# anxingle/AlphaPig

Hardware: AMD Instinct MI355X
Metric: self-play games/sec (15x15, n_playout=400) (higher is better)
Workload: dtype f32 (split operands on the bf16/fp16 matrix pipe, fp32 accumulate; <=1e-4 vs float64 oracle)

## Files before the change

alphapig_amd/csrc/apz_engine.hip:

```cpp
#include <hip/hip_runtime.h>

#include <algorithm>
#include <cmath>
#include <cstdio>
#include <cstdlib>
#include <cstring>
#include <map>
#include <mutex>
#include <string>
#include <vector>

#include "alphapig_hip.h"
#include "conv3x3_mfma.h"
#include "heads.h"
#include "trunk15_ring.h"
#include "trunk15_wino3.h"
#include "trunk15_wino3s.h"
#include "trunk15_wino3b.h"
#include "trunk15_wino3h.h"
#include "trunk15_wino3h16.h"
#include "conv8_split.h"
#include "conv8_small.h"
#include "wgrad_wino3.h"
#include "sampler.h"
// ... 35 lines not shown
    bool residual;
    float* wpk = nullptr;
    float* wpk12 = nullptr;
    float* upk2 = nullptr;
    float* upk3s = nullptr;
    void* upk3b = nullptr;
    void* upk3h = nullptr;
    float* bias3h = nullptr;
    void* wpk8h = nullptr;
    float* bias8h = nullptr;
    float* bias = nullptr;
};

struct Pending {
    int cls;
    hipEvent_t a, b;
    int launches;
};

}

struct apz_engine {
    apz_config cfg;
    int hw = 0, code_stride = 0, num_cu = 256, cmax = 0, clast = 0;
    hipStream_t stream = nullptr;
    std::vector<Param> params;
    std::vector<ConvLayer> convs;
    bool loaded = false;
    float *w6 = nullptr, *b6 = nullptr, *wfc_pk = nullptr, *bfc = nullptr, *wv = nullptr, *bv = nullptr;
    float* act[3] = {nullptr, nullptr, nullptr};
    float *planes = nullptr, *featp = nullptr, *featv = nullptr, *probs = nullptr, *values = nullptr, *fc_logits = nullptr;
    unsigned char* codes = nullptr;
    int *perm_s = nullptr, *perm_p = nullptr;
    float *h_planes = nullptr, *h_probs = nullptr, *h_values = nullptr;
    unsigned char* h_codes = nullptr;
    int last_n = 0;
    struct Slot {
        unsigned char* h_codes = nullptr;
        float *h_probs = nullptr, *h_values = nullptr;
        float *d_probs = nullptr, *d_values = nullptr;
        unsigned char* d_codes = nullptr;
        hipEvent_t done = nullptr;
        int n = 0;
        bool busy = false;
    } slots[APZ_MAX_SLOTS];
    std::map<long, hipGraphExec_t> fwd_graphs;
    std::map<long, int> fwd_seen;
    bool use_graphs = false;
    std::recursive_mutex submit_lock;
    bool ring = false;
    bool small8 = false;
    float* wfc_raw = nullptr;
    int act_ps = 0, act_rs = 0;
    bool lds_attr_set[44] = {false};
    int conv_lds_set[16] = {0};
    int32_t* smp_vis = nullptr;
    float* smp_pi = nullptr;
    int32_t* smp_mv = nullptr;
    uint64_t* smp_keys = nullptr;
    size_t smp_cap = 0;
    float* zeros256 = nullptr;
    double* bn_part = nullptr;
    float* wgw_scratch = nullptr;
    double* fold_ws = nullptr;
    float* head_scratch = nullptr;
    size_t head_scratch_floats = 0;
    size_t wgw_floats = 0;
    void* adam_tab = nullptr;
    size_t adam_cap = 0;
    float* wino_scratch[2] = {nullptr, nullptr};
    size_t wino_scratch_boards = 0;
    bool wgrad_attr_set[2] = {false, false};
    hipStream_t scratch_stream = nullptr;
    bool scratch_stream_valid = false;
    float* w3s_slabs = nullptr;
    unsigned* w3s_tickets = nullptr;
    unsigned w3s_epoch = 0;
    bool no_small_trunk = false;
    bool no_quarter_trunk = false;
    int trunk_arith = APZ_ARITH_F32;
    unsigned* ovf_host = nullptr;
    unsigned* ovf_dev = nullptr;
    unsigned* ovf_cur = nullptr;
    bool force_f32 = false;
    bool f16x2_k8 = false;
    long ovf_repeats = 0;
    int trunk_kernel = APZ_TRUNK_WINOGRAD;
    bool profiling = false;
    int prof_stride = 1, prof_phase = 0;
    bool prof_now = false;
    std::vector<Pending> pending;
    std::vector<hipEvent_t> free_events;
    double k_ms[APZ_K_COUNT] = {0};
    long k_cnt[APZ_K_COUNT] = {0};
};

namespace {

void add_param(apz_engine* e, const std::string& n, int64_t sz) { e->params.push_back({n, sz}); }

void build_tables(apz_engine* e) {
    const apz_config& c = e->cfg;
    const int hw = e->hw;
    auto conv_act = [&](const std::string& name, int cin, int cout, int k) {
        add_param(e, name + "_weight", (int64_t)cout * cin * k * k);
        add_param(e, name + "_bias", cout);
        add_param(e, name + "_gamma", cout);
        add_param(e, name + "_beta", cout);
        add_param(e, name + "_mean", cout);
        add_param(e, name + "_var", cout);
    };
    int last = 0;
    if (c.net_kind == APZ_NET_RESNET) {
        const int F = c.n_filter;
        conv_act("res_conv1", c.c_in, F, 3);
        e->convs.push_back({"res_conv1", "res_conv1", "_mean", "_var", true, c.c_in, (c.c_in + 3) / 4 * 4, F, false});
        for (int i = 1; i <= c.n_blocks; i++) {
            for (const char* ab : {"A", "B"}) {
                const std::string cn = std::string("conv") + ab + std::to_string(i);
                const std::string bn = std::string("bn") + ab + std::to_string(i);
                add_param(e, cn + "_weight", (int64_t)F * F * 9);
                add_param(e, cn + "_bias", F);
                add_param(e, bn + "_gamma", F);
                add_param(e, bn + "_beta", F);
                add_param(e, bn + "_moving_mean", F);
                add_param(e, bn + "_moving_var", F);
                e->convs.push_back({cn, bn, "_moving_mean", "_moving_var", false, F, F, F, ab[0] == 'B'});
            }
        }
        last = F;
    } else {
        static const char* names[6] = {"conv1", "conv2", "conv3", "conv4", "conv5", "conv_final"};
        static const int widths[6] = {64, 64, 128, 128, 256, 256};
        int prev = c.c_in;
        for (int i = 0; i < 6; i++) {
            conv_act(names[i], prev, widths[i], 3);
            e->convs.push_back({names[i], names[i], "_mean", "_var", true, prev, (prev + 3) / 4 * 4, widths[i], false});
            prev = widths[i];
// ... 168 lines not shown
        configured = true;
    }
    if (upk_small && n <= apz::Wino3S::MAX_BOARDS && !e->no_small_trunk) {
        if (!e->w3s_slabs) {
            HIP_TRY(hipMalloc((void**)&e->w3s_slabs, apz::Wino3S::slab_floats() * sizeof(float)));
            HIP_TRY(hipMalloc((void**)&e->w3s_tickets, apz::Wino3S::counters() * sizeof(unsigned)));
            e->w3s_epoch = 0;
        }
        if (++e->w3s_epoch == 0 || e->w3s_epoch == 1) {
            e->w3s_epoch = 1;
            HIP_TRY(hipMemsetAsync(e->w3s_tickets, 0, apz::Wino3S::counters() * sizeof(unsigned), e->stream));
        }
        hipLaunchKernelGGL((apz::trunk15_wino3s_kernel<RESID, RELU>), dim3(n * 16), dim3(256), apz::Wino3S::LDS_BYTES, e->stream, in,
                           upk_small, bias, RESID ? resid : nullptr, out, n, e->w3s_slabs, e->w3s_tickets, e->w3s_epoch);
        HIP_TRY(hipGetLastError());
        return APZ_OK;
    }
    for (int b0 = 0; b0 < n; b0 += WINO3_MAX_BOARDS) {
        const int nb = std::min(n - b0, WINO3_MAX_BOARDS);
        const size_t off = (size_t)b0 * T::C * T::GPLANE;
        bool quarter = false;
        const int grid = apz::wino3_grid(nb, e->num_cu, e->no_quarter_trunk ? nullptr : &quarter);
        if (quarter)
            hipLaunchKernelGGL((apz::trunk15_wino3_kernel<RESID, RELU, true>), dim3(grid), dim3(512), T::LDS_BYTES, e->stream,
                               in + off, upk, bias, RESID ? resid + off : nullptr, out + off, nb);
        else
            hipLaunchKernelGGL((apz::trunk15_wino3_kernel<RESID, RELU>), dim3(grid), dim3(512), T::LDS_BYTES, e->stream, in + off,
                               upk, bias, RESID ? resid + off : nullptr, out + off, nb);
    }
    HIP_TRY(hipGetLastError());
    return APZ_OK;
}

template <bool RESID>
int launch_wino3b_t(apz_engine* e, int attr_slot, const ConvLayer& L, const float* in, const float* resid, float* out, int n) {
    using T = apz::Wino3B;
    bool& configured = e->lds_attr_set[attr_slot];
    if (!configured) {
        HIP_TRY(hipFuncSetAttribute((const void*)apz::trunk15_wino3b_kernel<RESID, true>, hipFuncAttributeMaxDynamicSharedMemorySize,
                                    T::LDS_BYTES));
        configured = true;
    }
    for (int b0 = 0; b0 < n; b0 += WINO3_MAX_BOARDS) {
        const int nb = std::min(n - b0, WINO3_MAX_BOARDS);
        const size_t off = (size_t)b0 * T::C * T::GPLANE;
        const int grid = apz::wino3_grid(nb, e->num_cu);
        hipLaunchKernelGGL((apz::trunk15_wino3b_kernel<RESID, true>), dim3(grid), dim3(512), T::LDS_BYTES, e->stream, in + off,
                           (const void*)L.upk3b, L.bias, RESID ? resid + off : nullptr, out + off, nb);
    }
    HIP_TRY(hipGetLastError());
    return APZ_OK;
}

template <bool RESID, bool K16>
int launch_wino3h_t(apz_engine* e, int attr_slot, const ConvLayer& L, const float* in, const float* resid, float* out, int n) {
    using T = typename std::conditional<K16, apz::Wino3H16, apz::Wino3H>::type;
    const void* kern = K16 ? (const void*)apz::trunk15_wino3h16_kernel<RESID, true> : (const void*)apz::trunk15_wino3h_kernel<RESID, true>;
    bool& configured = e->lds_attr_set[attr_slot];
    if (!configured) {
        HIP_TRY(hipFuncSetAttribute(kern, hipFuncAttributeMaxDynamicSharedMemorySize, T::LDS_BYTES));
        configured = true;
    }
    for (int b0 = 0; b0 < n; b0 += WINO3_MAX_BOARDS) {
        const int nb = std::min(n - b0, WINO3_MAX_BOARDS);
        const size_t off = (size_t)b0 * T::C * T::GPLANE;
        const int grid = apz::wino3_grid(nb, e->num_cu);
        if constexpr (K16)
            hipLaunchKernelGGL((apz::trunk15_wino3h16_kernel<RESID, true>), dim3(grid), dim3(512), T::LDS_BYTES, e->stream, in + off,
                               (const void*)L.upk3h, L.bias3h, RESID ? resid + off : nullptr, out + off, nb, e->ovf_cur, nullptr, 0);
        else
            hipLaunchKernelGGL((apz::trunk15_wino3h_kernel<RESID, true>), dim3(grid), dim3(512), T::LDS_BYTES, e->stream, in + off,
                               (const void*)L.upk3h, L.bias3h, RESID ? resid + off : nullptr, out + off, nb, e->ovf_cur);
    }
    HIP_TRY(hipGetLastError());
    return APZ_OK;
}

int launch_trunk_wino3(apz_engine* e, const ConvLayer& L, const float* in, const float* resid, float* out, int n) {
    if (e->trunk_arith == APZ_ARITH_F16X2 && !e->force_f32 && L.upk3h && e->ovf_cur &&
        (n > apz::Wino3S::MAX_BOARDS || e->no_small_trunk)) {
        if (e->f16x2_k8) {
            if (resid) return launch_wino3h_t<true, false>(e, 32, L, in, resid, out, n);
            return launch_wino3h_t<false, false>(e, 33, L, in, resid, out, n);
        }
        if (resid) return launch_wino3h_t<true, true>(e, 36, L, in, resid, out, n);
        return launch_wino3h_t<false, true>(e, 37, L, in, resid, out, n);
    }
    if (e->trunk_arith == APZ_ARITH_BF16X3 && L.upk3b && (n > apz::Wino3S::MAX_BOARDS || e->no_small_trunk)) {
        if (resid) return launch_wino3b_t<true>(e, 26, L, in, resid, out, n);
        return launch_wino3b_t<false>(e, 27, L, in, resid, out, n);
    }
    if (resid) return launch_wino3_t<true, true>(e, 6, in, L.upk2, L.bias, resid, out, n, L.upk3s);
    return launch_wino3_t<false, true>(e, 7, in, L.upk2, L.bias, nullptr, out, n, L.upk3s);
}

int launch_trunk_ring(apz_engine* e, const ConvLayer& L, const float* in, const float* resid, float* out, int n) {
    if (e->trunk_kernel == APZ_TRUNK_WINOGRAD && L.upk2) return launch_trunk_wino3(e, L, in, resid, out, n);
    return launch_trunk_ring_t<4>(e, L, in, resid, out, n);
}

template <int C4, int CIN, bool CODES>
int launch_stem15_t(apz_engine* e, const ConvLayer& L, const float* in, float* out, int n) {
    constexpr int lds = apz::stem15_lds_bytes<C4>();
    bool& configured = e->lds_attr_set[(C4 == 1 ? 2 : 3) + (CODES ? 22 : 0)];
    if (!configured) {
        HIP_TRY(hipFuncSetAttribute((const void*)apz::stem15_kernel<C4, CIN, CODES>, hipFuncAttributeMaxDynamicSharedMemorySize,
                                    lds));
        configured = true;
    }
    const int grid = std::min(n, e->num_cu * (C4 == 1 ? 4 : 2));
    hipLaunchKernelGGL((apz::stem15_kernel<C4, CIN, CODES>), dim3(grid), dim3(256), lds, e->stream, in, L.wpk, L.bias, out, n,
                       L.cin, (int)e->code_stride);
    HIP_TRY(hipGetLastError());
    return APZ_OK;
}

int launch_stem15(apz_engine* e, const ConvLayer& L, const float* in, float* out, int n, const unsigned char* codes = nullptr) {
    if (codes) {
        if (L.cin == 4) return launch_stem15_t<1, 4, true>(e, L, (const float*)codes, out, n);
        if (L.cin == 9) return launch_stem15_t<3, 9, true>(e, L, (const float*)codes, out, n);
    } else {
        if (L.cin == 4) return launch_stem15_t<1, 4, false>(e, L, in, out, n);
        if (L.cin == 9) return launch_stem15_t<3, 9, false>(e, L, in, out, n);
    }
    return fail(APZ_E_UNSUPPORTED, "stem15: C_in must be 4 or 9");
}

template <bool RESID, bool CODES>
int launch_conv8_t(apz_engine* e, const ConvLayer& L, const float* in, const float* resid, float* out, int n) {
    using T = apz::Conv8;
    bool& configured = e->lds_attr_set[28 + (RESID ? 1 : 0) + (CODES ? 2 : 0)];
    if (!configured) {
        HIP_TRY(hipFuncSetAttribute((const void*)apz::conv8_kernel<RESID, CODES>, hipFuncAttributeMaxDynamicSharedMemorySize,
                                    T::LDS_BYTES));
        configured = true;
    }
    const long items = (long)n * (L.cout / 16);
    const int grid = (int)std::min<long>(items, 2L * e->num_cu);
// ... 254 lines not shown
    }
    void* host[] = {e->h_planes, e->h_probs, e->h_values, e->h_codes};
    for (void* p : host)
        if (p) hipHostFree(p);
    if (e->stream) hipStreamDestroy(e->stream);
    delete e;
}

apz_engine* apz_create(const apz_config* cfg) {
    if (!cfg || cfg->height < 1 || cfg->width < 1 || cfg->max_batch < 1 || (cfg->c_in != 9 && cfg->c_in != 4)) {
        fail(APZ_E_ARG, "bad config (c_in must be 9 or 4)");
        return nullptr;
    }
    if (!((cfg->height == 15 && cfg->width == 15) || (cfg->height == 8 && cfg->width == 8))) {
        fail(APZ_E_UNSUPPORTED, "HIP kernels are instantiated for 15x15 and 8x8 boards");
        return nullptr;
    }
    if (cfg->net_kind == APZ_NET_RESNET &&
        ((cfg->n_filter != 64 && cfg->n_filter != 128 && cfg->n_filter != 256) || cfg->n_blocks < 0)) {
        fail(APZ_E_UNSUPPORTED, "n_filter must be 64, 128 or 256");
        return nullptr;
    }
    if (cfg->net_kind != APZ_NET_RESNET && cfg->net_kind != APZ_NET_SIMPLE) {
        fail(APZ_E_ARG, "unknown net_kind");
        return nullptr;
    }
    int ndev = 0;
    if (hipGetDeviceCount(&ndev) != hipSuccess || ndev < 1) {
        fail(APZ_E_HIP, "no HIP device: libalphapig_hip needs an AMD GPU (there is no CPU fallback)");
        return nullptr;
    }
    if (cfg->device < 0 || cfg->device >= ndev) {
        fail(APZ_E_ARG, "device ordinal out of range");
        return nullptr;
    }
    apz_engine* e = new apz_engine();
    e->cfg = *cfg;
    e->hw = cfg->height * cfg->width;
    e->code_stride = (e->hw + 1 + 15) / 16 * 16;
    build_tables(e);
    auto bail = [&](const char* what, hipError_t err) -> apz_engine* {
        fail(APZ_E_HIP, std::string(what) + ": " + hipGetErrorString(err));
        apz_destroy(e);
        return nullptr;
    };
    hipError_t err;
    if ((err = hipSetDevice(cfg->device)) != hipSuccess) return bail("hipSetDevice", err);
    hipDeviceProp_t prop;
    if ((err = hipGetDeviceProperties(&prop, cfg->device)) != hipSuccess) return bail("hipGetDeviceProperties", err);
    e->num_cu = prop.multiProcessorCount > 0 ? prop.multiProcessorCount : 256;
    {
        const char* k8 = getenv("APZ_F16X2_K8");
        e->f16x2_k8 = k8 && atoi(k8) != 0;
    }
    if ((err = hipStreamCreateWithFlags(&e->stream, hipStreamNonBlocking)) != hipSuccess)
        return bail("hipStreamCreate", err);
    e->ring = cfg->net_kind == APZ_NET_RESNET && cfg->height == 15 && cfg->width == 15 && cfg->n_filter == 128;
    e->small8 = cfg->height == 8 && cfg->width == 8;
    e->act_ps = e->ring ? apz::Trunk15::GPLANE : e->hw;
    e->act_rs = e->ring ? apz::Trunk15::GROW : cfg->width;
    const size_t B = cfg->max_batch, hw = e->hw;
    const size_t act_bytes = B * e->cmax * (size_t)e->act_ps * sizeof(float);
    for (int i = 0; i < 3; i++)
    {
        if ((err = hipMalloc((void**)&e->act[i], act_bytes)) != hipSuccess) return bail("hipMalloc(act)", err);
        if ((err = hipMemset(e->act[i], 0, act_bytes)) != hipSuccess) return bail("hipMemset(act)", err);
    }
    if ((err = hipMalloc((void**)&e->planes, B * 9 * hw * sizeof(float))) != hipSuccess) return bail("hipMalloc", err);
    if ((err = hipMalloc((void**)&e->featp, B * 4 * hw * sizeof(float))) != hipSuccess) return bail("hipMalloc", err);
    if ((err = hipMalloc((void**)&e->featv, B * 2 * hw * sizeof(float))) != hipSuccess) return bail("hipMalloc", err);
    if ((err = hipMalloc((void**)&e->probs, B * hw * sizeof(float))) != hipSuccess) return bail("hipMalloc", err);
    if ((err = hipMalloc((void**)&e->fc_logits, B * ((hw + 15) / 16 * 16) * sizeof(float))) != hipSuccess) return bail("hipMalloc", err);
    if ((err = hipMalloc((void**)&e->values, B * sizeof(float))) != hipSuccess) return bail("hipMalloc", err);
    if ((err = hipMalloc((void**)&e->codes, B * e->code_stride)) != hipSuccess) return bail("hipMalloc", err);
    if ((err = hipMemset(e->codes, 0, B * e->code_stride)) != hipSuccess) return bail("hipMemset(codes)", err);
    if ((err = hipHostMalloc((void**)&e->h_planes, B * 9 * hw * sizeof(float))) != hipSuccess) return bail("hipHostMalloc", err);
    if ((err = hipHostMalloc((void**)&e->h_probs, B * hw * sizeof(float))) != hipSuccess) return bail("hipHostMalloc", err);
    if ((err = hipHostMalloc((void**)&e->h_values, B * sizeof(float))) != hipSuccess) return bail("hipHostMalloc", err);
    if ((err = hipHostMalloc((void**)&e->h_codes, B * e->code_stride)) != hipSuccess) return bail("hipHostMalloc", err);
    if (cfg->height == cfg->width) {
        std::vector<int> ps, pp;
        build_perms(cfg->height, ps, pp);
        if (upload(&e->perm_s, ps) || upload(&e->perm_p, pp)) {
            apz_destroy(e);
            return nullptr;
        }
    }
    return e;
}

int apz_param_count(apz_engine* e) { return e ? (int)e->params.size() : fail(APZ_E_ARG, "null engine"); }

const char* apz_param_name(apz_engine* e, int i) {
    if (!e || i < 0 || i >= (int)e->params.size()) return nullptr;
    return e->params[i].name.c_str();
}

int64_t apz_param_size(apz_engine* e, int i) {
    if (!e || i < 0 || i >= (int)e->params.size()) return -1;
    return e->params[i].size;
}

int apz_load_weights(apz_engine* e, const char* const* names, const float* const* ptrs, const int64_t* sizes, int n) {
    if (!e || !names || !ptrs || !sizes) return fail(APZ_E_ARG, "null argument");
    EngineLock guard(e->submit_lock);
    HIP_TRY(hipSetDevice(e->cfg.device));
// ... 667 lines not shown
    if (!e || !x_dev || !upk_dev || !y_dev || !stats_dev || n < 1) return fail(APZ_E_ARG, "bad argument");
    if (e->cfg.height != 15 || e->cfg.width != 15) return fail(APZ_E_UNSUPPORTED, "wino_conv: 15x15 boards only");
    if (n > WINO3_MAX_BOARDS) return fail(APZ_E_UNSUPPORTED, "wino_conv_stats: one launch (<= 16384 boards)");
    using T = apz::Wino3;
    EngineLock guard(e->submit_lock);
    HIP_TRY(hipSetDevice(e->cfg.device));
    if (!e->zeros256) {
        HIP_TRY(hipMalloc((void**)&e->zeros256, 256 * sizeof(float)));
        HIP_TRY(hipMemset(e->zeros256, 0, 256 * sizeof(float)));
    }
    StreamScope sc(e, stream);
    bool& configured = e->lds_attr_set[11];
    if (!configured) {
        HIP_TRY(hipFuncSetAttribute((const void*)apz::trunk15_wino3_kernel<false, false, false, true>,
                                    hipFuncAttributeMaxDynamicSharedMemorySize, T::LDS_BYTES));
        HIP_TRY(hipFuncSetAttribute((const void*)apz::trunk15_wino3_kernel<false, false, true, true>,
                                    hipFuncAttributeMaxDynamicSharedMemorySize, T::LDS_BYTES));
        configured = true;
    }
    const float* b = bias_dev ? (const float*)bias_dev : e->zeros256;
    bool quarter = false;
    const int grid = apz::wino3_grid(n, e->num_cu, e->no_quarter_trunk ? nullptr : &quarter);
    if (quarter)
        hipLaunchKernelGGL((apz::trunk15_wino3_kernel<false, false, true, true>), dim3(grid), dim3(512), T::LDS_BYTES, e->stream,
                           (const float*)x_dev, (const float*)upk_dev, b, (const float*)stats_dev, (float*)y_dev, n);
    else
        hipLaunchKernelGGL((apz::trunk15_wino3_kernel<false, false, false, true>), dim3(grid), dim3(512), T::LDS_BYTES, e->stream,
                           (const float*)x_dev, (const float*)upk_dev, b, (const float*)stats_dev, (float*)y_dev, n);
    HIP_TRY(hipGetLastError());
    return APZ_OK;
}

int apz_wino_conv(apz_engine* e, const void* x_dev, const void* upk_dev, const void* bias_dev, void* y_dev, int n, int relu,
                  int layout, void* stream) {
    return apz_wino_conv_add(e, x_dev, upk_dev, bias_dev, nullptr, y_dev, n, relu, layout, stream);
}

int64_t apz_wino3h_packed_size(void) { return (int64_t)(apz::Wino3H16::UPK_BYTES / 4); }

int apz_wino3h_pack_many(apz_engine* e, const void* w_dev, const void* b_dev, int count, void* upk_dev, void* bias_dev,
                         void* flag_dev, void* stream) {
    if (!e || !w_dev || !upk_dev || !bias_dev || count < 1 || count > 16384) return fail(APZ_E_ARG, "bad argument");
    EngineLock guard(e->submit_lock);
    HIP_TRY(hipSetDevice(e->cfg.device));
    StreamScope sc(e, stream);
    hipLaunchKernelGGL(apz::pack_wino3h16_many_kernel, dim3(128, 2 * count), dim3(128), 0, e->stream, (const float*)w_dev,
                       (const float*)b_dev, (unsigned short*)upk_dev, (float*)bias_dev, (unsigned*)flag_dev);
    HIP_TRY(hipGetLastError());
    return APZ_OK;
}

extern "C++" {
namespace {
template <int FORM, bool RESID>
int launch_wino3h16_train(apz_engine* e, int attr_slot, const void* x_dev, const void* upk_dev, const void* bias_dev,
                          const void* resid_dev, void* y_dev, int n, void* flag_dev, void* aux, int aux_n, void* stream) {
    if (!e || !x_dev || !upk_dev || !bias_dev || !y_dev || !aux || n < 1) return fail(APZ_E_ARG, "bad argument");
    if (e->cfg.height != 15 || e->cfg.width != 15) return fail(APZ_E_UNSUPPORTED, "wino3h: 15x15 boards only");
    if (n > WINO3_MAX_BOARDS) return fail(APZ_E_UNSUPPORTED, "wino3h: one launch (<= 16384 boards)");
    using T = apz::Wino3H16;
    const auto kern = apz::trunk15_wino3h16_kernel<RESID, false, FORM>;
    EngineLock guard(e->submit_lock);
    HIP_TRY(hipSetDevice(e->cfg.device));
    StreamScope sc(e, stream);
    bool& configured = e->lds_attr_set[attr_slot];
    if (!configured) {
        HIP_TRY(hipFuncSetAttribute((const void*)kern, hipFuncAttributeMaxDynamicSharedMemorySize, T::LDS_BYTES));
        configured = true;
    }
    hipLaunchKernelGGL(kern, dim3(apz::wino3_grid(n, e->num_cu)), dim3(512), T::LDS_BYTES, e->stream, (const float*)x_dev, upk_dev,
                       (const float*)bias_dev, (const float*)resid_dev, (float*)y_dev, n, (unsigned*)flag_dev, aux, aux_n);
    HIP_TRY(hipGetLastError());
    return APZ_OK;
}
}
}

int apz_wino3h_conv_stats(apz_engine* e, const void* x_dev, const void* upk_dev, const void* bias_dev, void* y_dev,
                          void* stats_dev, int n, void* flag_dev, void* stream) {
    return launch_wino3h16_train<apz::WINO3H16_STATS, false>(e, 40, x_dev, upk_dev, bias_dev, nullptr, y_dev, n, flag_dev,
                                                             stats_dev, 0, stream);
}

int apz_wino3h_conv_dgrad(apz_engine* e, const void* dy_dev, const void* upk_dev, const void* bias_dev, const void* add_dev,
                          void* dx_dev, int n, const void* dymax_dev, int dymax_count, void* flag_dev, void* stream) {
    if (dymax_count < 1) return fail(APZ_E_ARG, "bad argument");
    void* dm = const_cast<void*>(dymax_dev);
    if (add_dev)
        return launch_wino3h16_train<apz::WINO3H16_DGRAD, true>(e, 41, dy_dev, upk_dev, bias_dev, add_dev, dx_dev, n, flag_dev, dm,
                                                                dymax_count, stream);
    return launch_wino3h16_train<apz::WINO3H16_DGRAD, false>(e, 42, dy_dev, upk_dev, bias_dev, nullptr, dx_dev, n, flag_dev, dm,
                                                             dymax_count, stream);
}

namespace {
int wgrad_scratch(apz_engine* e, size_t floats) {
    if (floats > e->wgw_floats) {
        HIP_TRY(hipDeviceSynchronize());
        if (e->wgw_scratch) HIP_TRY(hipFree(e->wgw_scratch));
        e->wgw_scratch = nullptr;
        e->wgw_floats = 0;
        HIP_TRY(hipMalloc((void**)&e->wgw_scratch, floats * sizeof(float)));
        e->wgw_floats = floats;
    }
    return APZ_OK;
}
}

int apz_conv3x3_wgrad(apz_engine* e, const void* x_dev, const void* dy_dev, void* dw_dev, int n, int cin, int cout,
                      int layout, void* stream) {
    if (!e || !x_dev || !dy_dev || !dw_dev || n < 1 || cin < 1 || cout < 32 || cout % 32 || layout < 0 || layout > 1)
        return fail(APZ_E_ARG, "bad argument (C_out must be a multiple of 32)");
    if (layout == APZ_LAYOUT_ROWS16 && (e->cfg.height != 15 || e->cfg.width != 15))
        return fail(APZ_E_UNSUPPORTED, "padded-row layout: 15x15 boards only");
    EngineLock guard(e->submit_lock);
    HIP_TRY(hipSetDevice(e->cfg.device));
    StreamScope sc(e, stream);
    const int H = e->cfg.height, W = e->cfg.width;
    const int gx = cout / 32, gy = (cin + 63) / 64;
    int slices = std::max(1, std::min(n, (e->num_cu * 2) / std::max(1, gx * gy)));
    if (H == 15 && W == 15) {
        using G = apz::WgradGeo<15, 15>;
        if (!e->wgrad_attr_set[0]) {
            HIP_TRY(hipFuncSetAttribute((const void*)apz::conv3x3_wgrad_kernel<15, 15>,
                                        hipFuncAttributeMaxDynamicSharedMemorySize, G::LDS_BYTES));
            e->wgrad_attr_set[0] = true;
// ... 611 lines not shown
```

alphapig_amd/csrc/trunk15_wino3h16.h:

```cpp
#pragma once
#include <hip/hip_runtime.h>

#include <cmath>
#include <cstdint>
#include <type_traits>

#include "trunk15_wino3h.h"

namespace apz {

struct Wino3H16 {
    static constexpr int C = 128, CK = 16, NCHUNK = C / CK;
    static constexpr int GPLANE = 240;
    static constexpr int VTERM = 32 * 32, VPOS = 2 * VTERM, V_BYTES = 36 * VPOS;
    static constexpr int UNIT = 2 * 32 * 16;
    static constexpr size_t UPK_BYTES = (size_t)4 * 4 * NCHUNK * 9 * 2 * UNIT;
    static constexpr int BIAS_FLOATS = 256;
    static constexpr int MQ_FLOATS = 36 * 16 * 32;
    static constexpr int SROW = 20, SPLANE = 16 * SROW;
    static constexpr int STG_FLOATS = 8 * 4 * SPLANE;
    static constexpr int LDS_BYTES = 2 * V_BYTES;
    static_assert((MQ_FLOATS + STG_FLOATS) * 4 <= LDS_BYTES, "the epilogue area fits over V");
    static_assert(LDS_BYTES <= 160 * 1024, "LDS");
    static_assert(UPK_BYTES == Wino3H::UPK_BYTES, "same weight buffer as trunk15_wino3h.h");
    __host__ __device__ static size_t upk_offset(int co, int ci, int pos, int term) {
        const int i = pos / 6, k = pos % 6, ri = i / 3, ki = k / 3, p9 = 3 * (i % 3) + (k % 3);
        const int cog = co >> 5, r = co & 31, chunk = ci >> 4, half = (ci >> 3) & 1, w = 2 * ri + ki;
        return ((((size_t)(cog * 4 + w) * NCHUNK + chunk) * 9 + p9) * 2 + term) * UNIT + half * 512 + r * 16 + (ci & 7) * 2;
    }
    static float scale_for(double m) { return Wino3H::scale_for(m); }
};

#ifdef APZ_WINO3H_STAMPS
__device__ unsigned long long apz_wino3h16_stamps[4 * 8 * 12];
#endif

#ifndef APZH16_RING
#define APZH16_RING 3
#endif
#ifndef APZH16_RAW_SLOT
#define APZH16_RAW_SLOT 4
#endif

enum { WINO3H16_PLAIN = 0, WINO3H16_STATS = 1, WINO3H16_DGRAD = 2 };

__device__ __forceinline__ int wino3h16_dgrad_exponent(float m) {
    if (!(m > 0.f)) return 0;
    const int e = (int)((__builtin_bit_cast(unsigned, m) >> 23) & 255u);
    const int a = 134 - e;
    return a < -64 ? -64 : (a > 64 ? 64 : a);
}

template <bool RESID, bool RELU = true, int FORM = WINO3H16_PLAIN>
__global__ __launch_bounds__(512) void trunk15_wino3h16_kernel(const float* __restrict__ in, const void* __restrict__ upk,
                                                               const float* __restrict__ bias, const float* __restrict__ resid,
                                                               float* __restrict__ out, int n, unsigned* __restrict__ flag,
                                                               void* __restrict__ aux, int aux_n) {
    using T = Wino3H16;
    constexpr bool STATS = FORM == WINO3H16_STATS, DGRAD = FORM == WINO3H16_DGRAD;
    static_assert(FORM == WINO3H16_PLAIN || !RELU, "the training forms have no ReLU");
    static_assert(!STATS || !RESID, "STATS: bias only");
#ifdef APZ_WINO3H_STAMPS
    unsigned long long st_acc[12] = {0, 0, 0, 0, 0, 0, 0, 0, 0, 0, 0, 0};
    unsigned long long st_t = __builtin_readcyclecounter();
    const unsigned long long st_t0 = st_t, st_r0 = __builtin_amdgcn_s_memrealtime();
#define APZH16_STAMP(ph_)                                             \
    {                                                                 \
        const unsigned long long now_ = __builtin_readcyclecounter(); \
        st_acc[ph_] += now_ - st_t;                                   \
        st_t = now_;                                                  \
    }
#else
#define APZH16_STAMP(ph_)
#endif
    extern __shared__ __attribute__((aligned(16))) float lds[];
    char* vbase = reinterpret_cast<char*>(lds);
    float* mq = lds;
    float* stg = mq + T::MQ_FLOATS;

    const int tid = threadIdx.x, lane = tid & 63;
    const int wave = __builtin_amdgcn_readfirstlane(tid >> 6);

    const int npairs = (n + 1) >> 1, G_ = (int)gridDim.x, b_ = (int)blockIdx.x;
    const bool duo = (G_ & 15) == 0;
    const int pair0 = duo ? ((b_ >> 4) * 8 + (b_ & 7)) : b_;
    const int pstride = duo ? (G_ >> 1) : G_;
    const int h_fix = (b_ >> 3) & 1;
    const int np = pair0 < npairs ? (npairs - pair0 + pstride - 1) / pstride : 0;
    const int nitems = duo ? np : 2 * np;
    if (np == 0) return;
    auto item_pair = [&](int t) { return pair0 + (duo ? t : (t >> 1)) * pstride; };
    auto item_half = [&](int t) { return duo ? h_fix : (t & 1); };

    float xsc = 1.f, xisc = 1.f;
    if constexpr (DGRAD) {
        const float* pm = static_cast<const float*>(aux);
        float m = 0.f;
        for (int i = tid; i < aux_n; i += 512) m = fmaxf(m, fabsf(pm[i]));
#pragma unroll
        for (int off = 32; off > 0; off >>= 1) m = fmaxf(m, __shfl_xor(m, off, 64));
        if (lane == 0) lds[wave] = m;
        __syncthreads();
#pragma unroll
        for (int w = 0; w < 8; w++) m = fmaxf(m, lds[w]);
        const int a = __builtin_amdgcn_readfirstlane(wino3h16_dgrad_exponent(m));
        xsc = __builtin_bit_cast(float, (unsigned)(127 + a) << 23);
// ... 101 lines not shown
            else if constexpr (part == 2) {
                emit(vp + (j * 6 + 0) * T::VPOS, oo[0], oo[3]);
                emit(vp + (j * 6 + 1) * T::VPOS, oo[1], oo[4]);
            } else emit(vp + (j * 6 + 2) * T::VPOS, oo[2], oo[5]);
        }
    };
    auto transform = [&](int vpar) {
#define APZH16_TS(k) tslice(vpar, std::integral_constant<int, k>{});
        APZH16_TS(0) APZH16_TS(1) APZH16_TS(2) APZH16_TS(3) APZH16_TS(4) APZH16_TS(5) APZH16_TS(6) APZH16_TS(7) APZH16_TS(8)
        APZH16_TS(9) APZH16_TS(10) APZH16_TS(11) APZH16_TS(12) APZH16_TS(13) APZH16_TS(14) APZH16_TS(15) APZH16_TS(16)
        APZH16_TS(17) APZH16_TS(18) APZH16_TS(19) APZH16_TS(20) APZH16_TS(21) APZH16_TS(22) APZH16_TS(23) APZH16_TS(24)
        APZH16_TS(25) APZH16_TS(26)
#undef APZH16_TS
    };

    const int cc = wave >> 2, ri = (wave >> 1) & 1, ki = wave & 1, blk = wave & 3;
    const int r31 = lane & 31, hh = lane >> 5;
    const unsigned a_vo = lane * 16;
    const int wpos0 = 18 * ri + 3 * ki;
    auto pos_off = [](int p9) { return (6 * (p9 / 3) + (p9 % 3)) * T::VPOS; };

    static constexpr int RING = APZH16_RING;
    static_assert(18 % RING == 0 && RING >= 2, "ring slots must tile two chunks");
    f16x8 ah[RING], al[RING];
    auto unit_base = [&](int t, int c) {
        const int cog = 2 * item_half(t) + cc;
        return (unsigned)(((cog * 4 + blk) * T::NCHUNK + c) * 18) * T::UNIT;
    };
    unsigned ub_cur = 0, ub_nxt = 0;
    auto unit_pair_at = [&](unsigned base, int p9, int slot) {
        const int u = 2 * p9;
        ah[slot] = __builtin_bit_cast(f16x8, __builtin_amdgcn_raw_buffer_load_b128(r_u, a_vo + (unsigned)(u & 3) * T::UNIT,
                                                                                  base + (unsigned)(u >> 2) * 4u * T::UNIT, 0));
        al[slot] = __builtin_bit_cast(f16x8, __builtin_amdgcn_raw_buffer_load_b128(r_u, a_vo + (unsigned)((u + 1) & 3) * T::UNIT,
                                                                                  base + (unsigned)((u + 1) >> 2) * 4u * T::UNIT, 0));
    };
    auto unit_load = [&](int p9, int slot) {
        if (p9 < 9) unit_pair_at(ub_cur, p9, slot);
        else unit_pair_at(ub_nxt, p9 - 9, slot);
    };

    unsigned nonfinite = 0;

    ub_cur = ub_nxt = unit_base(0, 0);
#pragma unroll
    for (int u = 0; u < RING - 1; u++) unit_load(u, u);
    raw_load(0, 0);
    if (wave >= 4) __builtin_amdgcn_s_setprio(1);

    for (int t = 0; t < nitems; t++) {
        const int h = item_half(t);
        const int bd0 = 2 * item_pair(t);
        const bool two = bd0 + 1 < n;
        __syncthreads();
        APZH16_STAMP(5)
        transform(0);
        raw_load(t, 1);
        f32x16h acc[9];
#pragma unroll
        for (int p = 0; p < 9; p++)
#pragma unroll
            for (int v = 0; v < 16; v++) acc[p][v] = 0.f;
        APZH16_STAMP(0)

        f16x8 bfr[2];
        auto chunk = [&](int c, auto PAR, auto XF, auto LD) {
            constexpr int par = decltype(PAR)::value;
            constexpr bool xf = decltype(XF)::value, ld = decltype(LD)::value;
            __syncthreads();
            APZH16_STAMP(1)
            ub_cur = ub_nxt;
            ub_nxt = c + 1 < T::NCHUNK ? ub_cur + 18u * T::UNIT : (t + 1 < nitems ? unit_base(t + 1, 0) : ub_cur + 18u * T::UNIT);
            const char* vp = vbase + par * T::V_BYTES;
            int le = __builtin_amdgcn_mbcnt_hi(~0u, __builtin_amdgcn_mbcnt_lo(~0u, 0u));
            asm volatile("" : "+v"(le));
            const int fcol = le & 31;
            const int b_hi = wpos0 * T::VPOS + fcol * 32 + ((((le >> 5) & 1) ^ ((fcol >> 3) & 1)) * 16);
            const int b_lo = b_hi + T::VTERM;
            bfr[0] = *reinterpret_cast<const f16x8*>(vp + b_hi);
            bfr[1] = *reinterpret_cast<const f16x8*>(vp + b_lo);
#define APZH16_SLOT(k)                                                                                                   \
            {                                                                                                            \
                constexpr int p9 = (k), slot = (par * 9 + (k)) % RING;                                                   \
                                                                   \
                acc[p9] = __builtin_amdgcn_mfma_f32_32x32x16_f16(ah[slot], bfr[1], acc[p9], 0, 0, 0);                    \
                if (p9 + 1 < 9) bfr[1] = *reinterpret_cast<const f16x8*>(vp + b_lo + pos_off(p9 + 1));                   \
                acc[p9] = __builtin_amdgcn_mfma_f32_32x32x16_f16(al[slot], bfr[0], acc[p9], 0, 0, 0);                    \
                acc[p9] = __builtin_amdgcn_mfma_f32_32x32x16_f16(ah[slot], bfr[0], acc[p9], 0, 0, 0);                    \
                if (p9 + 1 < 9) bfr[0] = *reinterpret_cast<const f16x8*>(vp + b_hi + pos_off(p9 + 1));                   \
                if (xf) {                                                                                                \
                    tslice(1 - par, std::integral_constant<int, 3 * (k)>{});                                             \
                    tslice(1 - par, std::integral_constant<int, 3 * (k) + 1>{});                                         \
                    tslice(1 - par, std::integral_constant<int, 3 * (k) + 2>{});                                         \
                }                                                                                                        \
                if ((k) == APZH16_RAW_SLOT && ld) raw_load(t, c + 2);                                                    \
                             \
                unit_load((k) + RING - 1, (par * 9 + (k) + RING - 1) % RING);                                            \
                __builtin_amdgcn_sched_barrier(0);                                                                       \
            }
            APZH16_SLOT(0) APZH16_SLOT(1) APZH16_SLOT(2) APZH16_SLOT(3) APZH16_SLOT(4) APZH16_SLOT(5) APZH16_SLOT(6) APZH16_SLOT(7) APZH16_SLOT(8)
#undef APZH16_SLOT
            APZH16_STAMP(2)
        };
        using P0 = std::integral_constant<int, 0>;
        using P1 = std::integral_constant<int, 1>;
        using Y = std::true_type;
        using N = std::false_type;
        for (int c = 0; c < T::NCHUNK - 2; c += 2) {
            chunk(c, P0{}, Y{}, Y{});
            chunk(c + 1, P1{}, Y{}, Y{});
        }
        chunk(T::NCHUNK - 2, P0{}, Y{}, N{});
        chunk(T::NCHUNK - 1, P1{}, N{}, N{});

        const int cosel = lane >> 5;
        const int col = lane & 31, gbd = col >> 4, gtile = col & 15;
        const int gty = gtile >> 2, gtx = gtile & 3;
        float* sw = stg + wave * (4 * T::SPLANE);
        const int s_lin = (lane >> 2) * T::SROW + (lane & 3) * 4;
        const unsigned ep_vo = lane < 60 ? lane * 16 : 0x80000000u;
        auto row_chan = [&](int s, int row) { return (2 * h + (row >> 3)) * 32 + 8 * s + (row & 7); };
        f32x4 rs[4];
        auto resid_request = [&](int s) {
#pragma unroll
            for (int pl = 0; pl < 4; pl++) {
                const int bdp = bd0 + (pl & 1);
                const int bd = bdp < n ? bdp : n - 1;
                rs[pl] = bload(r_res, ep_vo, (unsigned)(bd * T::C + row_chan(s, 2 * wave + (pl >> 1))) * plane_b);
            }
        };
        if (RESID) resid_request(0);
        auto ep_step = [&](auto S_) {
            constexpr int s = decltype(S_)::value;
            __syncthreads();
            APZH16_STAMP(4)
            {
                float* mw = mq + wpos0 * 512 + (8 * cc + 4 * hh) * 32 + r31;
#pragma unroll
                for (int p9 = 0; p9 < 9; p9++)
#pragma unroll
                    for (int e4 = 0; e4 < 4; e4++) mw[(6 * (p9 / 3) + p9 % 3) * 512 + e4 * 32] = acc[p9][4 * s + e4];
            }
            if (RESID) {
#pragma unroll
                for (int pl = 0; pl < 4; pl++) *reinterpret_cast<f32x4*>(sw + pl * T::SPLANE + s_lin) = rs[pl];
            }
            if (s == 3 && t + 1 < nitems) raw_load(t + 1, 0);
            APZH16_STAMP(8)
            __syncthreads();
            APZH16_STAMP(10)
            {
                const int co16 = 2 * wave + cosel;
                const float* mp = mq + co16 * 32 + col;
                float hrow[6][4];
#pragma unroll
                for (int i = 0; i < 6; i++) {
                    float m[6];
#pragma unroll
                    for (int k = 0; k < 6; k++) m[k] = mp[(6 * i + k) * 512];
                    const float s12 = m[1] + m[2], d12 = m[1] - m[2], s34 = m[3] + m[4], d34 = m[3] - m[4];
                    hrow[i][0] = (m[0] + s12) + s34;
                    hrow[i][1] = __builtin_fmaf(2.f, d34, d12);
                    hrow[i][2] = __builtin_fmaf(4.f, s34, s12);
                    hrow[i][3] = __builtin_fmaf(8.f, d34, d12) + m[5];
                }
                if (RESID && s + 1 < 4) resid_request(s + 1);
                const int ch = row_chan(s, co16);
// ... 3 lines not shown
                f32x4 y[4];
#pragma unroll
                for (int ee = 0; ee < 4; ee++) {
                    const float s12 = hrow[1][ee] + hrow[2][ee], d12 = hrow[1][ee] - hrow[2][ee];
                    const float s34 = hrow[3][ee] + hrow[4][ee], d34 = hrow[3][ee] - hrow[4][ee];
                    y[0][ee] = (hrow[0][ee] + s12) + s34;
                    y[1][ee] = __builtin_fmaf(2.f, d34, d12);
                    y[2][ee] = __builtin_fmaf(4.f, s34, s12);
                    y[3][ee] = __builtin_fmaf(8.f, d34, d12) + hrow[5][ee];
                }
                float chk = 0.f;
                float r1[4], r2[4];
#pragma unroll
                for (int a = 0; a < 4; a++) {
                    f32x4 v;
#pragma unroll
                    for (int ee = 0; ee < 4; ee++) v[ee] = __builtin_fmaf(y[a][ee], is, bv);
                    if (RESID) v += *reinterpret_cast<const f32x4*>(sp + a * T::SROW);
                    chk += (v[0] + v[1]) + (v[2] + v[3]);
#pragma unroll
                    for (int ee = 0; ee < 4; ee++) v[ee] = RELU ? fmaxf(v[ee], 0.f) : v[ee];
                    if (gtx == 3) v[3] = 0.f;
                    *reinterpret_cast<f32x4*>(sp + a * T::SROW) = v;
                    if constexpr (STATS) {
                        r1[a] = (v[0] + v[1]) + (v[2] + v[3]);
                        r2[a] = (v[0] * v[0] + v[1] * v[1]) + (v[2] * v[2] + v[3] * v[3]);
                    }
                }
                nonfinite |= ((chk - chk) != 0.f) ? 1u : 0u;
                if constexpr (STATS) {
                    if (gty == 3) r1[3] = 0.f, r2[3] = 0.f;
                    const double d1 = (double)wino3_row16_sum((r1[0] + r1[1]) + (r1[2] + r1[3]));
                    const double d2 = (double)wino3_row16_sum((r2[0] + r2[1]) + (r2[2] + r2[3]));
                    const bool mine = gtile == 0 && (gbd == 0 || two);
                    typedef double f64x2 __attribute__((ext_vector_type(2)));
                    const unsigned so = (unsigned)(ch * n + bd0 + gbd) * 16u;
                    bstore(r_st, mine ? so : 0x80000000u, 0u, __builtin_bit_cast(f32x4, f64x2{d1, d2}));
                }
            }
            APZH16_STAMP(9)
            wave_lds_fence();
#pragma unroll
            for (int pl = 0; pl < 4; pl++) {
                const f32x4 pv = *reinterpret_cast<const f32x4*>(sw + pl * T::SPLANE + s_lin);
                const unsigned vo = ((pl & 1) == 0 || two) ? ep_vo : 0x80000000u;
                bstore(r_out, vo, (unsigned)((bd0 + (pl & 1)) * T::C + row_chan(s, 2 * wave + (pl >> 1))) * plane_b, pv);
            }
            APZH16_STAMP(3)
        };
        ep_step(std::integral_constant<int, 0>{});
        ep_step(std::integral_constant<int, 1>{});
        ep_step(std::integral_constant<int, 2>{});
        ep_step(std::integral_constant<int, 3>{});
    }
    if (nonfinite && flag) *reinterpret_cast<volatile unsigned*>(flag) = 1u;
#ifdef APZ_WINO3H_STAMPS
    st_acc[7] = __builtin_readcyclecounter() - st_t0;
    st_acc[6] = __builtin_amdgcn_s_memrealtime() - st_r0;
    if (lane == 0 && blockIdx.x < 4)
        for (int i = 0; i < 12; i++) apz_wino3h16_stamps[(blockIdx.x * 8 + wave) * 12 + i] = st_acc[i];
#endif
#undef APZH16_STAMP
}

}
```

Measured before the change: 14.88.

## Add direct-store epilogue variant to wino3h16 trunk kernel, keep staged path as EPI0

```diff
diff --git a/alphapig_amd/csrc/apz_engine.hip b/alphapig_amd/csrc/apz_engine.hip
--- a/alphapig_amd/csrc/apz_engine.hip
+++ b/alphapig_amd/csrc/apz_engine.hip
@@ -111,7 +111,7 @@
     bool small8 = false;
     float* wfc_raw = nullptr;
     int act_ps = 0, act_rs = 0;
-    bool lds_attr_set[44] = {false};
+    bool lds_attr_set[49] = {false};
     int conv_lds_set[16] = {0};
     int32_t* smp_vis = nullptr;
     float* smp_pi = nullptr;
@@ -143,6 +143,7 @@
     unsigned* ovf_cur = nullptr;
     bool force_f32 = false;
     bool f16x2_k8 = false;
+    bool wino3h16_epi0 = false;
     long ovf_repeats = 0;
     int trunk_kernel = APZ_TRUNK_WINOGRAD;
     bool profiling = false;
@@ -417,10 +418,11 @@
     return APZ_OK;
 }
 
-template <bool RESID, bool K16>
+template <bool RESID, bool K16, bool EPI0 = false>
 int launch_wino3h_t(apz_engine* e, int attr_slot, const ConvLayer& L, const float* in, const float* resid, float* out, int n) {
     using T = typename std::conditional<K16, apz::Wino3H16, apz::Wino3H>::type;
-    const void* kern = K16 ? (const void*)apz::trunk15_wino3h16_kernel<RESID, true> : (const void*)apz::trunk15_wino3h_kernel<RESID, true>;
+    const void* kern = K16 ? (const void*)apz::trunk15_wino3h16_kernel<RESID, true, apz::WINO3H16_PLAIN, EPI0>
+                           : (const void*)apz::trunk15_wino3h_kernel<RESID, true>;
     bool& configured = e->lds_attr_set[attr_slot];
     if (!configured) {
         HIP_TRY(hipFuncSetAttribute(kern, hipFuncAttributeMaxDynamicSharedMemorySize, T::LDS_BYTES));
@@ -431,7 +433,7 @@
         const size_t off = (size_t)b0 * T::C * T::GPLANE;
         const int grid = apz::wino3_grid(nb, e->num_cu);
         if constexpr (K16)
-            hipLaunchKernelGGL((apz::trunk15_wino3h16_kernel<RESID, true>), dim3(grid), dim3(512), T::LDS_BYTES, e->stream, in + off,
+            hipLaunchKernelGGL((apz::trunk15_wino3h16_kernel<RESID, true, apz::WINO3H16_PLAIN, EPI0>), dim3(grid), dim3(512), T::LDS_BYTES, e->stream, in + off,
                                (const void*)L.upk3h, L.bias3h, RESID ? resid + off : nullptr, out + off, nb, e->ovf_cur, nullptr, 0);
         else
             hipLaunchKernelGGL((apz::trunk15_wino3h_kernel<RESID, true>), dim3(grid), dim3(512), T::LDS_BYTES, e->stream, in + off,
@@ -448,7 +450,8 @@
             if (resid) return launch_wino3h_t<true, false>(e, 32, L, in, resid, out, n);
             return launch_wino3h_t<false, false>(e, 33, L, in, resid, out, n);
         }
-        if (resid) return launch_wino3h_t<true, true>(e, 36, L, in, resid, out, n);
+        if (resid) return launch_wino3h_t<true, true, true>(e, 44, L, in, resid, out, n);
+        if (e->wino3h16_epi0) return launch_wino3h_t<false, true, true>(e, 45, L, in, resid, out, n);
         return launch_wino3h_t<false, true>(e, 37, L, in, resid, out, n);
     }
     if (e->trunk_arith == APZ_ARITH_BF16X3 && L.upk3b && (n > apz::Wino3S::MAX_BOARDS || e->no_small_trunk)) {
@@ -809,6 +812,8 @@
     {
         const char* k8 = getenv("APZ_F16X2_K8");
         e->f16x2_k8 = k8 && atoi(k8) != 0;
+        const char* epi0 = getenv("APZ_WINO3H16_EPI0");
+        e->wino3h16_epi0 = epi0 && atoi(epi0) != 0;
     }
     if ((err = hipStreamCreateWithFlags(&e->stream, hipStreamNonBlocking)) != hipSuccess)
         return bail("hipStreamCreate", err);
@@ -1582,14 +1587,14 @@
 
 extern "C++" {
 namespace {
-template <int FORM, bool RESID>
-int launch_wino3h16_train(apz_engine* e, int attr_slot, const void* x_dev, const void* upk_dev, const void* bias_dev,
+template <int FORM, bool RESID, bool EPI0>
+int launch_wino3h16_train_t(apz_engine* e, int attr_slot, const void* x_dev, const void* upk_dev, const void* bias_dev,
                           const void* resid_dev, void* y_dev, int n, void* flag_dev, void* aux, int aux_n, void* stream) {
     if (!e || !x_dev || !upk_dev || !bias_dev || !y_dev || !aux || n < 1) return fail(APZ_E_ARG, "bad argument");
     if (e->cfg.height != 15 || e->cfg.width != 15) return fail(APZ_E_UNSUPPORTED, "wino3h: 15x15 boards only");
     if (n > WINO3_MAX_BOARDS) return fail(APZ_E_UNSUPPORTED, "wino3h: one launch (<= 16384 boards)");
     using T = apz::Wino3H16;
-    const auto kern = apz::trunk15_wino3h16_kernel<RESID, false, FORM>;
+    const auto kern = apz::trunk15_wino3h16_kernel<RESID, false, FORM, EPI0>;
     EngineLock guard(e->submit_lock);
     HIP_TRY(hipSetDevice(e->cfg.device));
     StreamScope sc(e, stream);
@@ -1602,6 +1607,15 @@
                        (const float*)bias_dev, (const float*)resid_dev, (float*)y_dev, n, (unsigned*)flag_dev, aux, aux_n);
     HIP_TRY(hipGetLastError());
     return APZ_OK;
+}
+template <int FORM, bool RESID>
+int launch_wino3h16_train(apz_engine* e, int attr_slot, const void* x_dev, const void* upk_dev, const void* bias_dev,
+                          const void* resid_dev, void* y_dev, int n, void* flag_dev, void* aux, int aux_n, void* stream) {
+    if (e && (e->wino3h16_epi0 || RESID))
+        return launch_wino3h16_train_t<FORM, RESID, true>(e, attr_slot + 6, x_dev, upk_dev, bias_dev, resid_dev, y_dev, n, flag_dev,
+                                                          aux, aux_n, stream);
+    return launch_wino3h16_train_t<FORM, RESID, false>(e, attr_slot, x_dev, upk_dev, bias_dev, resid_dev, y_dev, n, flag_dev, aux,
+                                                       aux_n, stream);
 }
 }
 }
diff --git a/alphapig_amd/csrc/trunk15_wino3h16.h b/alphapig_amd/csrc/trunk15_wino3h16.h
--- a/alphapig_amd/csrc/trunk15_wino3h16.h
+++ b/alphapig_amd/csrc/trunk15_wino3h16.h
@@ -20,7 +20,8 @@
     static constexpr int SROW = 20, SPLANE = 16 * SROW;
     static constexpr int STG_FLOATS = 8 * 4 * SPLANE;
     static constexpr int LDS_BYTES = 2 * V_BYTES;
-    static_assert((MQ_FLOATS + STG_FLOATS) * 4 <= LDS_BYTES, "the epilogue area fits over V");
+    static_assert((MQ_FLOATS + STG_FLOATS) * 4 <= LDS_BYTES, "the EPI0 epilogue area fits over V");
+    static_assert(MQ_FLOATS * 4 == V_BYTES, "M buffer s & 1 lies exactly over V[s & 1]");
     static_assert(LDS_BYTES <= 160 * 1024, "LDS");
     static_assert(UPK_BYTES == Wino3H::UPK_BYTES, "same weight buffer as trunk15_wino3h.h");
     __host__ __device__ static size_t upk_offset(int co, int ci, int pos, int term) {
@@ -51,7 +52,7 @@
     return a < -64 ? -64 : (a > 64 ? 64 : a);
 }
 
-template <bool RESID, bool RELU = true, int FORM = WINO3H16_PLAIN>
+template <bool RESID, bool RELU = true, int FORM = WINO3H16_PLAIN, bool EPI0 = false>
 __global__ __launch_bounds__(512) void trunk15_wino3h16_kernel(const float* __restrict__ in, const void* __restrict__ upk,
                                                                const float* __restrict__ bias, const float* __restrict__ resid,
                                                                float* __restrict__ out, int n, unsigned* __restrict__ flag,
@@ -259,7 +260,7 @@
         const int h = item_half(t);
         const int bd0 = 2 * item_pair(t);
         const bool two = bd0 + 1 < n;
-        __syncthreads();
+        if (EPI0 || t == 0) __syncthreads();
         APZH16_STAMP(5)
         transform(0);
         raw_load(t, 1);
@@ -320,6 +321,7 @@
         chunk(T::NCHUNK - 2, P0{}, Y{}, N{});
         chunk(T::NCHUNK - 1, P1{}, N{}, N{});
 
+        if constexpr (EPI0) {
         const int cosel = lane >> 5;
         const int col = lane & 31, gbd = col >> 4, gtile = col & 15;
         const int gty = gtile >> 2, gtx = gtile & 3;
@@ -429,6 +431,104 @@
         ep_step(std::integral_constant<int, 1>{});
         ep_step(std::integral_constant<int, 2>{});
         ep_step(std::integral_constant<int, 3>{});
+        } else {
+        const int cosel = lane >> 5;
+        const int col = lane & 31, gbd = col >> 4, gtile = col & 15;
+        const int gty = gtile >> 2, gtx = gtile & 3;
+        const int co16 = 2 * wave + cosel;
+        auto row_chan = [&](int s, int row) { return (2 * h + (row >> 3)) * 32 + 8 * s + (row & 7); };
+        const unsigned t_vo0 = (unsigned)((4 * gty * 16 + 4 * gtx) * 4);
+        auto t_vo = [&](int a) { return (a == 3 && gty == 3) ? 0x80000000u : t_vo0 + (unsigned)a * 64u; };
+        f32x4 rs[4];
+        auto resid_request = [&](int s) {
+            const int bd = bd0 + gbd < n ? bd0 + gbd : n - 1;
+            const unsigned so = (unsigned)(bd * T::C + row_chan(s, co16)) * plane_b;
+#pragma unroll
+            for (int a = 0; a < 4; a++) rs[a] = bload(r_res, t_vo(a), so);
+        };
+        if (RESID) resid_request(0);
+        auto ep_step = [&](auto S_) {
+            constexpr int s = decltype(S_)::value;
+            float* mb = mq + (s & 1) * T::MQ_FLOATS;
+            APZH16_STAMP(4)
+            {
+                float* mw = mb + wpos0 * 512 + (8 * cc + 4 * hh) * 32 + r31;
+#pragma unroll
+                for (int p9 = 0; p9 < 9; p9++)
+#pragma unroll
+                    for (int e4 = 0; e4 < 4; e4++) mw[(6 * (p9 / 3) + p9 % 3) * 512 + e4 * 32] = acc[p9][4 * s + e4];
+            }
+            if (s == 3 && t + 1 < nitems) raw_load(t + 1, 0);
+            APZH16_STAMP(8)
+            __syncthreads();
+            APZH16_STAMP(10)
+            {
+                const float* mp = mb + co16 * 32 + col;
+                float hrow[6][4];
+#pragma unroll
+                for (int i = 0; i < 6; i++) {
+                    float m[6];
+#pragma unroll
+                    for (int k = 0; k < 6; k++) m[k] = mp[(6 * i + k) * 512];
+                    const float s12 = m[1] + m[2], d12 = m[1] - m[2], s34 = m[3] + m[4], d34 = m[3] - m[4];
+                    hrow[i][0] = (m[0] + s12) + s34;
+                    hrow[i][1] = __builtin_fmaf(2.f, d34, d12);
+                    hrow[i][2] = __builtin_fmaf(4.f, s34, s12);
+                    hrow[i][3] = __builtin_fmaf(8.f, d34, d12) + m[5];
+                }
+                const int ch = row_chan(s, co16);
+                const float bv = bias[ch];
+                const float is = DGRAD ? bias[128 + ch] * xisc : bias[128 + ch];
+                f32x4 y[4];
+#pragma unroll
+                for (int ee = 0; ee < 4; ee++) {
+                    const float s12 = hrow[1][ee] + hrow[2][ee], d12 = hrow[1][ee] - hrow[2][ee];
+                    const float s34 = hrow[3][ee] + hrow[4][ee], d34 = hrow[3][ee] - hrow[4][ee];
+                    y[0][ee] = (hrow[0][ee] + s12) + s34;
+                    y[1][ee] = __builtin_fmaf(2.f, d34, d12);
+                    y[2][ee] = __builtin_fmaf(4.f, s34, s12);
+                    y[3][ee] = __builtin_fmaf(8.f, d34, d12) + hrow[5][ee];
+                }
+                const unsigned so = (unsigned)((bd0 + gbd) * T::C + ch) * plane_b;
+                float chk = 0.f;
+                float r1[4], r2[4];
+#pragma unroll
+                for (int a = 0; a < 4; a++) {
+                    f32x4& v = y[a];
+#pragma unroll
+                    for (int ee = 0; ee < 4; ee++) v[ee] = __builtin_fmaf(y[a][ee], is, bv);
+                    if (RESID) v += rs[a];
+                    chk += (v[0] + v[1]) + (v[2] + v[3]);
+#pragma unroll
+                    for (int ee = 0; ee < 4; ee++) v[ee] = RELU ? fmaxf(v[ee], 0.f) : v[ee];
+                    if (gtx == 3) v[3] = 0.f;
+                    if constexpr (STATS) {
+                        r1[a] = (v[0] + v[1]) + (v[2] + v[3]);
+                        r2[a] = (v[0] * v[0] + v[1] * v[1]) + (v[2] * v[2] + v[3] * v[3]);
+                    }
+                }
+                nonfinite |= ((chk - chk) != 0.f) ? 1u : 0u;
+                if (RESID && s + 1 < 4) resid_request(s + 1);
+#pragma unroll
+                for (int a = 0; a < 4; a++)
+                    bstore(r_out, (gbd == 0 || two) ? t_vo(a) : 0x80000000u, so, y[a]);
+                if constexpr (STATS) {
+                    if (gty == 3) r1[3] = 0.f, r2[3] = 0.f;
+                    const double d1 = (double)wino3_row16_sum((r1[0] + r1[1]) + (r1[2] + r1[3]));
+                    const double d2 = (double)wino3_row16_sum((r2[0] + r2[1]) + (r2[2] + r2[3]));
+                    const bool mine = gtile == 0 && (gbd == 0 || two);
+                    typedef double f64x2 __attribute__((ext_vector_type(2)));
+                    const unsigned sso = (unsigned)(ch * n + bd0 + gbd) * 16u;
+                    bstore(r_st, mine ? sso : 0x80000000u, 0u, __builtin_bit_cast(f32x4, f64x2{d1, d2}));
+                }
+            }
+            APZH16_STAMP(9)
+        };
+        ep_step(std::integral_constant<int, 0>{});
+        ep_step(std::integral_constant<int, 1>{});
+        ep_step(std::integral_constant<int, 2>{});
+        ep_step(std::integral_constant<int, 3>{});
+        }
     }
     if (nonfinite && flag) *reinterpret_cast<volatile unsigned*>(flag) = 1u;
 #ifdef APZ_WINO3H_STAMPS
```

Result: no change. 14.81, median of 2 (-0.4%).
